# conceptofmind/vit-flax

Hardware: NVIDIA B200
Metric: images/sec ViT-B/16 224 bf16 fwd at 1/2/4/8 B200; % tensor-pipe peak (higher is better)
Workload: dtype bf16

## Files before the change

vit_flax_b200/csrc/attention_tc5.cu:

```cuda
#include <cstdlib>

#include "common.h"
#include "ptx.cuh"

namespace vb {

#ifdef VITB200_TRACE
__device__ long long g_trace[12][64];
#define TRACE(ev, i) do { if (blockIdx.x == 0 && (i) < 64) g_trace[ev][i] = clock64(); } while (0)
#else
#define TRACE(ev, i) do { } while (0)
#endif

namespace {

constexpr int DH = 64;
constexpr int QT = 128;
constexpr int NT = 512;
constexpr int Q_BYTES = QT * 128;
constexpr int O_BYTES = QT * 128;

constexpr int QS = 4;
constexpr int KS = 2;

// ... 26 lines not shown
        fma_f32x2(pack_f32x2(__uint_as_float(r[2 * j]), __uint_as_float(r[2 * j + 1])), sl2x2, mnegx2);
    float a0, a1;
    unpack_f32x2(a2, a0, a1);
    const float p0 = ex2_approx(a0), p1 = ex2_approx(a1);
    if (j & 1) lb = add_f32x2(lb, pack_f32x2(p0, p1));
    else la = add_f32x2(la, pack_f32x2(p0, p1));
    pp[j] = pack2<kDT>(p0, p1);
  }
}

template <int kDT, int KP>
__global__ void __launch_bounds__(NT, 1)
attention_tc5_kernel(const __grid_constant__ CUtensorMap tmQ,
                     const __grid_constant__ CUtensorMap tmKV,
                     const __grid_constant__ CUtensorMap tmO,
                     int T, int heads, int nqt, int items, int turns, float* __restrict__ lse_out) {
  using L = Smem<KP>;
  constexpr uint32_t SLOT_COLS = KP <= 128 ? 128 : 208;
  constexpr uint32_t O_COL = 2 * SLOT_COLS;
  static_assert(O_COL + DH <= 512, "TMEM budget");
  extern __shared__ uint8_t smem_raw[];
  const uint32_t base = (smem_u32(smem_raw) + 1023u) & ~1023u;
  uint8_t* gbase = smem_raw + (base - smem_u32(smem_raw));
  const uint32_t sQ = base + L::OFF_Q, sK = base + L::OFF_K, sV = base + L::OFF_V, sO = base + L::OFF_O;
  const uint32_t bars = base + L::OFF_BAR;
  auto q_full = [&](int s) { return bars + 8u * (0 + s); };
  auto q_empty = [&](int s) { return bars + 8u * (4 + s); };
  auto k_full = [&](int s) { return bars + 8u * (8 + s); };
  auto v_full = [&](int s) { return bars + 8u * (10 + s); };
  auto k_empty = [&](int s) { return bars + 8u * (12 + s); };
  auto v_empty = [&](int s) { return bars + 8u * (14 + s); };
// ... 14 lines not shown
  const int n = int(last - first);

  if (warp == 0 && lane == 0) {
    prefetch_tmap(&tmQ);
    prefetch_tmap(&tmKV);
    prefetch_tmap(&tmO);
  }
  if (warp == 1 && lane == 0) {
    for (int s = 0; s < QS; ++s) {
      mbar_init(q_full(s), 1);
      mbar_init(q_empty(s), 1);
    }
    for (int s = 0; s < 2; ++s) {
      mbar_init(k_full(s), 1);
      mbar_init(v_full(s), 1);
      mbar_init(k_empty(s), nqt);
      mbar_init(v_empty(s), nqt);
      mbar_init(s_ready(s), 1);
      for (int g = 0; g < 4; ++g) mbar_init(p_part(s, g), 4);
      mbar_init(o_ready(s), 1);
    }
    mbar_init(o_free, 4);
    for (int q = 0; q < 4; ++q) mbar_init(xu_done(q), 1);
    fence_barrier_init();
  }
  if (warp == 2) tmem_alloc<1>(tmem_slot, 512);
  tc_fence_before();
  __syncthreads();
  tc_fence_after();
  const uint32_t tmem_base = *tmem_slot_ptr;
  pdl_launch_dependents();
  pdl_wait();

  const int bh0 = int(first / nqt);
  if (warp == 0) {
    if (elect_one()) {
      for (int i = 0; i < n; ++i) {
        const int64_t item = first + i;
        const int bh = int(item / nqt), qt = int(item - int64_t(bh) * nqt);
        const int b = bh / heads, h = bh - b * heads;
        const int e = bh - bh0, es = e & 1;
        const uint32_t eph = (e >> 1) & 1;
        const bool first_of_bh = (i == 0) || (qt == 0);
        if (first_of_bh) {
          mbar_wait(k_empty(es), eph ^ 1u);
          mbar_arrive_expect_tx(k_full(es), L::KV_BYTES);
          tma_load_3d(sK + es * L::KV_BYTES, &tmKV, k_full(es), inner + h * DH, 0, b);
        }
        const int qs = i & (QS - 1);
        mbar_wait(q_empty(qs), ((i / QS) & 1) ^ 1u);
        TRACE(0, i);
        mbar_arrive_expect_tx(q_full(qs), Q_BYTES);
        tma_load_3d(sQ + qs * Q_BYTES, &tmQ, q_full(qs), h * DH, qt * QT, b);
        if (first_of_bh) {
          mbar_wait(v_empty(es), eph ^ 1u);
          TRACE(1, i);
          mbar_arrive_expect_tx(v_full(es), L::KV_BYTES);
          tma_load_3d(sV + es * L::KV_BYTES, &tmKV, v_full(es), 2 * inner + h * DH, 0, b);
        }
      }
    }
    __syncwarp();
  } else if (warp == 1 || warp == 3) {
    if (elect_one()) {
      constexpr int fmt = kDT == DT_F16 ? 0 : 1;
      constexpr uint32_t idesc_s = umma_idesc_16(QT, KP, fmt, 0);
      constexpr uint32_t idesc_o = umma_idesc_16(QT, DH, fmt, 1);
      constexpr int NPARTS = KP >= 128 ? KP / 64 : 1;
      const int s = warp == 1 ? 0 : 1;
      const uint32_t d_s = tmem_base + s * SLOT_COLS, d_o = tmem_base + O_COL;
      const int first_lo = int(first % nqt);
      auto meta = [&](int i, int& es, uint32_t& eph, int& missing) {
        const int t = first_lo + i;
        const int e = t / nqt;
        es = e & 1;
        eph = (e >> 1) & 1;
        missing = i == 0 ? first_lo : 0;
      };
      auto issue_s = [&](int i) {
        int es, missing; uint32_t eph;
        meta(i, es, eph, missing);
        const int qs = i & (QS - 1);
        mbar_wait(q_full(qs), (i / QS) & 1);
        mbar_wait(k_full(es), eph);
        TRACE(2, i);
        tc_fence_after();
        const uint32_t q0 = sQ + qs * Q_BYTES, k0 = sK + es * L::KV_BYTES;
#pragma unroll
        for (int k = 0; k < DH / 16; ++k)
          umma_bf16_ss<1>(d_s, umma_desc_k_sw128(q0 + k * 32), umma_desc_k_sw128(k0 + k * 32), idesc_s,
                          k != 0 ? 1u : 0u);
        umma_commit(q_empty(qs));
        umma_commit(k_empty(es));
        for (int j = 0; j < missing; ++j) mbar_arrive(k_empty(es));
        umma_commit(s_ready(s));
      };
      if (s < n) issue_s(s);
      for (int i = s; i < n; i += 2) {
        int es, missing; uint32_t eph;
        meta(i, es, eph, missing);
        const uint32_t ph = (i >> 1) & 1;
        const uint32_t v0 = sV + es * L::KV_BYTES;
#pragma unroll
        for (int g = 0; g < NPARTS; ++g) {
          mbar_wait(p_part(s, g), ph);
          if (g == 0) {
            mbar_wait(v_full(es), eph);
            mbar_wait(o_free, uint32_t(i & 1) ^ 1u);
            TRACE(3, i);
          }
          tc_fence_after();
          constexpr int KSTEPS = KP / 16;
          const int k_end = g == NPARTS - 1 ? KSTEPS : 4 * g + 4;
#pragma unroll
          for (int kk = 4 * g; kk < k_end; ++kk)
            umma_bf16_ts(d_o, d_s + kk * 8, umma_desc_mn_sw128(v0 + kk * 2048), idesc_o, kk != 0 ? 1u : 0u);
        }
        umma_commit(v_empty(es));
        for (int j = 0; j < missing; ++j) mbar_arrive(v_empty(es));
        umma_commit(o_ready(s));
        if (i + 2 < n) issue_s(i + 2);
      }
    }
    __syncwarp();
  } else if (warp >= 4 && warp < 12) {
    const int w = warp - 4;
    const int q = w & 3;
    const int grp = w >> 2;
    const int row = q * 32 + lane;
    const uint32_t t_slot = tmem_base + (uint32_t(q * 32) << 16) + uint32_t(grp * SLOT_COLS);
    const float sl2 = 0.125f * 1.4426950408889634f;
    constexpr int NFULL = KP / 32, TAIL = KP % 32;
    constexpr int KMIN = KP == 208 ? 128 : (KP == 128 ? 64 : 0);
    static_assert(TAIL == 0 || TAIL == 16, "key block = n*32 (+16)");
    constexpr int NPARTS = KP >= 128 ? KP / 64 : 1;
    static_assert(NPARTS <= 4 && 2 * NPARTS <= NFULL, "parts are pairs of 32-key chunks");

    for (int i = grp; i < n; i += 2) {
      const uint32_t ph = (i >> 1) & 1;
      const int64_t item = first + i;
      const int bh = int(item / nqt), qt = int(item - int64_t(bh) * nqt);
      const bool active = qt * QT + q * 32 < T;
      if (q == 0 && lane == 0) TRACE(4, i);
      mbar_wait(s_ready(grp), ph);
      if (q == 0 && lane == 0) TRACE(5, i);
      tc_fence_after();
      if (active) {
        uint32_t r[2][32];
        float mx = -INFINITY;
        tmem_ld_32x32b_x32p(t_slot, r[0]);
        tmem_ld_wait();
#pragma unroll
        for (int c = 0; c < NFULL; ++c) {
          if (c + 1 < NFULL) tmem_ld_32x32b_x32p(t_slot + (c + 1) * 32, r[(c + 1) & 1]);
          else if (TAIL) tmem_ld_32x32b_x16(t_slot + (c + 1) * 32, r[(c + 1) & 1]);
          uint32_t* rc = r[c & 1];
          if (c * 32 + 32 > KMIN && c * 32 + 32 > T) {
// ... 38 lines not shown
            if (lane == 0) mbar_arrive(p_part(grp, c / 2 - 1));
          }
          tmem_st_32x32b_x16(t_slot + c * 16, pp);
          if (c + 1 == turns) { __syncwarp(); if (lane == 0) mbar_arrive(xu_done(q)); }
        }
        if constexpr (TAIL != 0) {
          uint32_t pp[8];
          softmax_chunk<kDT, 16, true>(r[NFULL & 1], pp, NFULL * 32, T, sl2x2, mnegx2, la, lb);
          tmem_st_32x32b_x8(t_slot + NFULL * 16, pp);
        }
        if (turns > NFULL) { __syncwarp(); if (lane == 0) mbar_arrive(xu_done(q)); }
        if (q == 0 && lane == 0) TRACE(11, i);
        float l0, l1;
        unpack_f32x2(add_f32x2(la, lb), l0, l1);
        inv_sh[(i & 3) * 128 + row] = 1.0f / (l0 + l1);
        if (lse_out != nullptr && qt * QT + row < T) lse_out[int64_t(bh) * T + qt * QT + row] = __log2f(l0 + l1) - mneg;
        tmem_st_wait();
        tc_fence_before();
        __syncwarp();
        if (lane == 0) mbar_arrive(p_part(grp, NPARTS - 1));
      } else {
        if (turns) {
          mbar_wait(xu_done(q), uint32_t(i & 1) ^ 1u);
          if (lane == 0) mbar_arrive(xu_done(q));
        }
        tc_fence_before();
        __syncwarp();
        if (lane == 0) {
#pragma unroll
          for (int g = 0; g < NPARTS; ++g) mbar_arrive(p_part(grp, g));
        }
      }
      if (q == 0 && lane == 0) TRACE(7, i);
    }
  } else if (warp >= 12) {
    const int q = warp & 3;
    const int row = q * 32 + lane;
    const bool leader = (q == 0 && lane == 0);
    const uint32_t t_lane = tmem_base + (uint32_t(q * 32) << 16);
    for (int i = 0; i < n; ++i) {
      const int s = i & 1;
      const uint32_t ph = (i >> 1) & 1;
      const int64_t item = first + i;
      const int bh = int(item / nqt), qt = int(item - int64_t(bh) * nqt);
      const int b = bh / heads, h = bh - b * heads;
      const bool active = qt * QT + q * 32 < T;
      const uint32_t sOi = sO + uint32_t(i & 1) * O_BYTES;
      if (leader) TRACE(8, i);
      mbar_wait(o_ready(s), ph);
      tc_fence_after();
      uint32_t o[64];
      float inv = 0.f;
      if (active) {
        tmem_ld_32x32b_x32p(t_lane + O_COL, o);
        tmem_ld_32x32b_x32p(t_lane + O_COL + 32, o + 32);
        inv = inv_sh[(i & 3) * 128 + row];
        tmem_ld_wait();
      }
      tc_fence_before();
      __syncwarp();
      if (lane == 0) mbar_arrive(o_free);
      if (active) {
#pragma unroll
        for (int g = 0; g < 8; ++g) {
          st_shared_v4(sOi + uint32_t(row) * 128u + (uint32_t(g ^ (row & 7)) << 4),
                       pack2<kDT>(__uint_as_float(o[g * 8 + 0]) * inv, __uint_as_float(o[g * 8 + 1]) * inv),
                       pack2<kDT>(__uint_as_float(o[g * 8 + 2]) * inv, __uint_as_float(o[g * 8 + 3]) * inv),
                       pack2<kDT>(__uint_as_float(o[g * 8 + 4]) * inv, __uint_as_float(o[g * 8 + 5]) * inv),
                       pack2<kDT>(__uint_as_float(o[g * 8 + 6]) * inv, __uint_as_float(o[g * 8 + 7]) * inv));
        }
      }
      fence_proxy_async_smem();
      if (leader) tma_store_wait_read<0>();
      named_bar_sync(1, 128);
      if (leader) {
        tma_store_3d(&tmO, sOi, h * DH, qt * QT, b);
        tma_store_commit();
        TRACE(10, i);
      }
    }
    if (leader) tma_store_wait<0>();
  }

  tc_fence_before();
  __syncthreads();
  if (warp == 2) {
    tc_fence_after();
    tmem_dealloc<1>(tmem_base, 512);
  }
}

int attn_turns() {
  static int v = -1;
  if (v < 0) {
    const char* e = getenv("VITB200_ATTN_TURNS");
    v = (e && e[0] >= '0' && e[0] <= '9') ? e[0] - '0' : -1;
  }
  return v;
}

template <int kDT, int KP>
int launch_kp(cudaStream_t stream, const void* qkv, void* out, int batch, int T, int heads, float* lse, int q_tiles) {
  using L = Smem<KP>;
  static PerDevice<bool> configured_on;
  if (bool& configured = configured_on.here(); !configured) {
    VB_CUDA(cudaFuncSetAttribute(attention_tc5_kernel<kDT, KP>, cudaFuncAttributeMaxDynamicSharedMemorySize, L::TOTAL));
    configured = true;
  }
  const int inner = heads * DH;
  CUtensorMap tq, tkv, to;
  int rc;
  if ((rc = make_tmap_3d_16(&tq, qkv, batch, T, 3 * inner, 3 * inner, QT, kDT))) return rc;
  if ((rc = make_tmap_3d_16(&tkv, qkv, batch, T, 3 * inner, 3 * inner, KP, kDT))) return rc;
  if ((rc = make_tmap_3d_16(&to, out, batch, T, inner, inner, QT, kDT))) return rc;
  const int nqt = q_tiles > 0 && q_tiles < ceil_div(T, QT) ? q_tiles : ceil_div(T, QT);
  const int64_t items64 = int64_t(batch) * heads * nqt;
  if (items64 > 0x7fffffff) return fail(VITB200_ERR_INVALID, "attention: too many work items");
  const int items = int(items64);
  const int grid = items < sm_count() ? items : sm_count();
  VB_CUDA(launch_kernel(attention_tc5_kernel<kDT, KP>, dim3(grid), dim3(NT), L::TOTAL, stream, 1,
                        tq, tkv, to, T, heads, nqt, items, attn_turns(), lse));
  VB_LAUNCH_CHECK("attention_tc5_kernel");
  return 0;
}

template <int kDT>
int launch_dt(cudaStream_t stream, const void* qkv, void* out, int batch, int T, int heads, float* lse, int q_tiles) {
  if (T <= 64) return launch_kp<kDT, 64>(stream, qkv, out, batch, T, heads, lse, q_tiles);
  if (T <= 128) return launch_kp<kDT, 128>(stream, qkv, out, batch, T, heads, lse, q_tiles);
  return launch_kp<kDT, 208>(stream, qkv, out, batch, T, heads, lse, q_tiles);
}

}

#ifdef VITB200_TRACE
}
extern "C" int vitb200_debug_attention_trace(long long* host, int n) {
  return cudaMemcpyFromSymbol(host, vb::g_trace, sizeof(long long) * (n < 12 * 64 ? n : 12 * 64)) == cudaSuccess ? 0 : -2;
}
namespace vb {
#endif

bool attention_tc5_supports(int T) { return T >= 1 && T <= 208; }

int launch_attention_tc5(cudaStream_t stream, const void* qkv, void* out, int batch, int T, int heads,
// ... 10 lines not shown
```

vit_flax_b200/csrc/common.h:

```cpp
#pragma once
#include <cuda.h>
#include <cuda_runtime.h>
#include <cuda_bf16.h>
#include <stdint.h>
#include <string>

#include "../../include/vitb200.h"
#include "ptx.cuh"

namespace vb {

void set_error(const std::string& msg);
int fail(int code, const std::string& msg);
int cuda_fail(cudaError_t e, const char* what);
void count_launch(int n = 1);
const std::string& last_error_ref();
int64_t launch_count();

#define VB_CUDA(expr)                                              \
  do {                                                             \
    cudaError_t _e = (expr);                                       \
    if (_e != cudaSuccess) return ::vb::cuda_fail(_e, #expr);      \
  } while (0)

// ... 38 lines not shown
    ++na;
  }
  if (pdl_enabled()) {
    attr[na].id = cudaLaunchAttributeProgrammaticStreamSerialization;
    attr[na].val.programmaticStreamSerializationAllowed = 1;
    ++na;
  }
  cfg.attrs = attr;
  cfg.numAttrs = unsigned(na);
  return cudaLaunchKernelEx(&cfg, kernel, KArgs(args)...);
}

int make_tmap_2d(CUtensorMap* out, const void* base, int64_t rows, int64_t cols, int64_t ld,
                 int box_rows, int dt, int box_bytes = 128);
int make_tmap_3d_16(CUtensorMap* out, const void* base, int64_t batch, int64_t rows, int64_t cols,
                    int64_t ld, int box_rows, int dt);

int make_tmap_im2col_patches(CUtensorMap* out, const float* images, int64_t batch, int H, int W, int C, int ph, int pw,
                             int pixels);

constexpr int GEMM_BM = 128;
constexpr int GEMM_BN = 256;
constexpr int GEMM_BK = 64;

int launch_gemm_tc(cudaStream_t stream, const CUtensorMap& tmA, const CUtensorMap& tmB,
                   const CUtensorMap* tmC, const float* bias, void* C, int M, int N, int K,
                   int epilogue, const float* aux, int tokens_per_image, int dtype, int cta_group,
                   const Dropout& drop = Dropout(), int cls_off = 1, const float* cls = nullptr,
                   const LnFold& ln = LnFold(), const float* wscale = nullptr);
int launch_fold_layernorm(cudaStream_t stream, const float* W, const float* gamma, const float* beta, const float* bias,
                          void* Wt, float* c, float* d, int K, int N, int Kpad, int dtype, float* scratch);
// ... 92 lines not shown
```

vit_flax_b200/csrc/ptx.cuh:

```cuda
#pragma once
#include <cuda_runtime.h>
#include <cuda_bf16.h>
#include <cuda_fp16.h>
#include <stdint.h>
#include <stdio.h>

namespace vb {

__device__ __forceinline__ uint32_t smem_u32(const void* p) {
  return static_cast<uint32_t>(__cvta_generic_to_shared(p));
}
__device__ __forceinline__ uint32_t lane_id() { return threadIdx.x & 31u; }
__device__ __forceinline__ bool elect_one() {
  uint32_t pred;
  asm volatile("{\n\t.reg .pred p;\n\telect.sync _|p, 0xffffffff;\n\tselp.u32 %0, 1, 0, p;\n\t}" : "=r"(pred));
  return pred != 0;
}

__device__ __forceinline__ void pdl_wait() { asm volatile("griddepcontrol.wait;" ::: "memory"); }
__device__ __forceinline__ void pdl_launch_dependents() {
  asm volatile("griddepcontrol.launch_dependents;" ::: "memory");
}

__device__ __forceinline__ void mbar_init(uint32_t bar, uint32_t count) {
// ... 107 lines not shown
  asm volatile("cp.async.bulk.tensor.2d.global.shared::cta.bulk_group [%0, {%2, %3}], [%1];"
               ::"l"(reinterpret_cast<uint64_t>(tmap)), "r"(src), "r"(c0), "r"(c1) : "memory");
}
__device__ __forceinline__ void tma_reduce_add_2d(const void* tmap, uint32_t src, int32_t c0, int32_t c1) {
  asm volatile("cp.reduce.async.bulk.tensor.2d.global.shared::cta.add.tile.bulk_group [%0, {%2, %3}], [%1];"
               ::"l"(reinterpret_cast<uint64_t>(tmap)), "r"(src), "r"(c0), "r"(c1) : "memory");
}
__device__ __forceinline__ void tma_store_3d(const void* tmap, uint32_t src, int32_t c0, int32_t c1, int32_t c2) {
  asm volatile("cp.async.bulk.tensor.3d.global.shared::cta.bulk_group [%0, {%2, %3, %4}], [%1];"
               ::"l"(reinterpret_cast<uint64_t>(tmap)), "r"(src), "r"(c0), "r"(c1), "r"(c2) : "memory");
}
__device__ __forceinline__ void tma_load_3d(uint32_t dst, const void* tmap, uint32_t bar,
                                            int32_t c0, int32_t c1, int32_t c2) {
  asm volatile(
      "cp.async.bulk.tensor.3d.shared::cluster.global.mbarrier::complete_tx::bytes"
      " [%0], [%1, {%3, %4, %5}], [%2];"
      ::"r"(dst), "l"(reinterpret_cast<uint64_t>(tmap)), "r"(bar), "r"(c0), "r"(c1), "r"(c2)
      : "memory");
}
__device__ __forceinline__ void tma_load_im2col_5d(uint32_t dst, const void* tmap, uint32_t bar, int32_t c, int32_t w,
                                                   int32_t h, int32_t d, int32_t n, uint16_t w_off, uint16_t h_off,
                                                   uint16_t d_off) {
  asm volatile(
      "cp.async.bulk.tensor.5d.shared::cluster.global.im2col.mbarrier::complete_tx::bytes"
      " [%0], [%1, {%3, %4, %5, %6, %7}], [%2], {%8, %9, %10};"
      ::"r"(dst), "l"(reinterpret_cast<uint64_t>(tmap)), "r"(bar), "r"(c), "r"(w), "r"(h), "r"(d), "r"(n), "h"(w_off),
        "h"(h_off), "h"(d_off)
      : "memory");
}
__device__ __forceinline__ void tma_store_commit() { asm volatile("cp.async.bulk.commit_group;" ::: "memory"); }
// ... 164 lines not shown

__device__ __forceinline__ uint64_t umma_desc_k_sw128(uint32_t addr) {
  return static_cast<uint64_t>((addr & 0x3FFFFu) >> 4)
         | (1ull << 16)
         | (64ull << 32)
         | (1ull << 46)
         | (2ull << 61);
}
__device__ __forceinline__ uint64_t umma_desc_mn_sw128(uint32_t addr) {
  return static_cast<uint64_t>((addr & 0x3FFFFu) >> 4) | (1ull << 16) | (64ull << 32) |
         (1ull << 46) | (2ull << 61);
}
__device__ __forceinline__ uint64_t umma_desc_mn_sw128_wide(uint32_t addr, uint32_t lbo_bytes) {
  return static_cast<uint64_t>((addr & 0x3FFFFu) >> 4) | (static_cast<uint64_t>(lbo_bytes >> 4) << 16) |
         (64ull << 32) | (1ull << 46) | (2ull << 61);
}
constexpr uint32_t UMMA_DESC_HI_SW128 = 0x40004040u;
__device__ __forceinline__ uint32_t umma_desc_lo(uint32_t addr, uint32_t lbo_bytes = 16) {
  return ((addr & 0x3FFFFu) >> 4) | ((lbo_bytes >> 4) << 16);
}
__device__ __forceinline__ void umma_bf16_ss_lo(uint32_t d_tmem, uint32_t a_lo, uint32_t b_lo, uint32_t idesc, uint32_t accumulate) {
  asm volatile(
      "{\n\t.reg .pred p;\n\t.reg .b64 da, db;\n\t"
      "setp.ne.b32 p, %4, 0;\n\t"
      "mov.b64 da, {%1, %5};\n\t"
      "mov.b64 db, {%2, %5};\n\t"
      "tcgen05.mma.cta_group::1.kind::f16 [%0], da, db, %3, p;\n\t}"
      ::"r"(d_tmem), "r"(a_lo), "r"(b_lo), "r"(idesc), "r"(accumulate), "r"(UMMA_DESC_HI_SW128) : "memory");
}

// ... 131 lines not shown
```

vit_flax_b200/csrc/runtime.cu:

```cuda
#include <atomic>
#include <cstdlib>
#include <mutex>

#include "common.h"

namespace vb {

namespace {
thread_local std::string g_last_error;
std::atomic<int64_t> g_launches{0};

typedef CUresult (*EncodeTiledFn)(CUtensorMap*, CUtensorMapDataType, cuuint32_t, void*,
                                  const cuuint64_t*, const cuuint64_t*, const cuuint32_t*,
                                  const cuuint32_t*, CUtensorMapInterleave, CUtensorMapSwizzle,
                                  CUtensorMapL2promotion, CUtensorMapFloatOOBfill);
EncodeTiledFn g_encode = nullptr;
std::once_flag g_encode_once;
typedef CUresult (*EncodeIm2colFn)(CUtensorMap*, CUtensorMapDataType, cuuint32_t, void*, const cuuint64_t*,
                                   const cuuint64_t*, const int*, const int*, cuuint32_t, cuuint32_t, const cuuint32_t*,
                                   CUtensorMapInterleave, CUtensorMapSwizzle, CUtensorMapL2promotion, CUtensorMapFloatOOBfill);
EncodeIm2colFn g_encode_im2col = nullptr;
std::once_flag g_encode_im2col_once;
}

// ... 60 lines not shown
  if (box_rows < 1 || box_rows > 256) return fail(VITB200_ERR_INVALID, "TMA box rows out of range");
  if (box_bytes != 128 && box_bytes != 64) return fail(VITB200_ERR_INVALID, "TMA box width must be 64 or 128 bytes");
  cuuint64_t gdim[2] = {static_cast<cuuint64_t>(cols), static_cast<cuuint64_t>(rows)};
  cuuint64_t gstride[1] = {static_cast<cuuint64_t>(ld) * esz};
  cuuint32_t box[2] = {static_cast<cuuint32_t>(box_bytes / esz), static_cast<cuuint32_t>(box_rows)};
  cuuint32_t estr[2] = {1u, 1u};
  CUresult r = g_encode(out, tmap_type(dt), 2, const_cast<void*>(base), gdim, gstride, box, estr,
                        CU_TENSOR_MAP_INTERLEAVE_NONE, box_bytes == 64 ? CU_TENSOR_MAP_SWIZZLE_64B : CU_TENSOR_MAP_SWIZZLE_128B,
                        CU_TENSOR_MAP_L2_PROMOTION_L2_256B, CU_TENSOR_MAP_FLOAT_OOB_FILL_NONE);
  if (r != CUDA_SUCCESS)
    return fail(VITB200_ERR_CUDA, "cuTensorMapEncodeTiled failed with CUresult " + std::to_string(int(r)));
  return 0;
}

int make_tmap_3d_16(CUtensorMap* out, const void* base, int64_t batch, int64_t rows, int64_t cols,
                    int64_t ld, int box_rows, int dt) {
  if (!load_encoder()) return fail(VITB200_ERR_CUDA, "cuTensorMapEncodeTiled entry point unavailable");
  if ((reinterpret_cast<uintptr_t>(base) & 15) != 0 || (ld * 2) % 16 != 0)
    return fail(VITB200_ERR_INVALID, "TMA operand must be 16-byte aligned with a 16-byte row pitch");
  if (box_rows < 1 || box_rows > 256) return fail(VITB200_ERR_INVALID, "TMA box rows out of range");
  cuuint64_t gdim[3] = {static_cast<cuuint64_t>(cols), static_cast<cuuint64_t>(rows), static_cast<cuuint64_t>(batch)};
  cuuint64_t gstride[2] = {static_cast<cuuint64_t>(ld) * 2, static_cast<cuuint64_t>(ld) * 2 * static_cast<cuuint64_t>(rows)};
  cuuint32_t box[3] = {64u, static_cast<cuuint32_t>(box_rows), 1u};
  cuuint32_t estr[3] = {1u, 1u, 1u};
  CUresult r = g_encode(out, tmap_type(dt), 3, const_cast<void*>(base), gdim, gstride, box, estr,
                        CU_TENSOR_MAP_INTERLEAVE_NONE, CU_TENSOR_MAP_SWIZZLE_128B,
                        CU_TENSOR_MAP_L2_PROMOTION_L2_256B, CU_TENSOR_MAP_FLOAT_OOB_FILL_NONE);
  if (r != CUDA_SUCCESS)
    return fail(VITB200_ERR_CUDA, "cuTensorMapEncodeTiled(3d) failed with CUresult " + std::to_string(int(r)));
  return 0;
}

int make_tmap_im2col_patches(CUtensorMap* out, const float* images, int64_t batch, int H, int W, int C, int ph, int pw,
                             int pixels) {
  std::call_once(g_encode_im2col_once, [] {
    void* fn = nullptr;
    cudaDriverEntryPointQueryResult q;
    if (cudaGetDriverEntryPoint("cuTensorMapEncodeIm2col", &fn, cudaEnableDefault, &q) == cudaSuccess &&
        q == cudaDriverEntryPointSuccess)
      g_encode_im2col = reinterpret_cast<EncodeIm2colFn>(fn);
  });
// ... 22 lines not shown
```

Baseline: 28840.

## Add two-CTA cluster attention kernel splitting each head across a CTA pair

Adds an attention kernel for ViT's 197-token sequences in which a two-CTA cluster handles one (batch, head). It uses cta_group::2 UMMA with M=256: each CTA loads half of K and half of V's columns, and P is staged through shared memory for the PV product. The existing single-CTA kernel loses its multi-q-tile path and now does one q tile per head item; the pair kernel runs whenever q_tiles != 1. The aim is to avoid the duplicated K/V loads and the partial second q tile of the per-q-tile scheme and to use the larger 2-SM MMA shape. The cost is cross-CTA mbarrier synchronisation and new SW32/SW64 descriptor layouts, which bring correctness risk.

```diff
diff --git a/vit_flax_b200/csrc/attention_tc5.cu b/vit_flax_b200/csrc/attention_tc5.cu
--- a/vit_flax_b200/csrc/attention_tc5.cu
+++ b/vit_flax_b200/csrc/attention_tc5.cu
@@ -64,7 +64,7 @@
 attention_tc5_kernel(const __grid_constant__ CUtensorMap tmQ,
                      const __grid_constant__ CUtensorMap tmKV,
                      const __grid_constant__ CUtensorMap tmO,
-                     int T, int heads, int nqt, int items, int turns, float* __restrict__ lse_out) {
+                     int T, int heads, int items, int turns, float* __restrict__ lse_out) {
   using L = Smem<KP>;
   constexpr uint32_t SLOT_COLS = KP <= 128 ? 128 : 208;
   constexpr uint32_t O_COL = 2 * SLOT_COLS;
@@ -109,8 +109,8 @@
     for (int s = 0; s < 2; ++s) {
       mbar_init(k_full(s), 1);
       mbar_init(v_full(s), 1);
-      mbar_init(k_empty(s), nqt);
-      mbar_init(v_empty(s), nqt);
+      mbar_init(k_empty(s), 1);
+      mbar_init(v_empty(s), 1);
       mbar_init(s_ready(s), 1);
       for (int g = 0; g < 4; ++g) mbar_init(p_part(s, g), 4);
       mbar_init(o_ready(s), 1);
@@ -127,32 +127,24 @@
   pdl_launch_dependents();
   pdl_wait();
 
-  const int bh0 = int(first / nqt);
   if (warp == 0) {
     if (elect_one()) {
       for (int i = 0; i < n; ++i) {
-        const int64_t item = first + i;
-        const int bh = int(item / nqt), qt = int(item - int64_t(bh) * nqt);
-        const int b = bh / heads, h = bh - b * heads;
-        const int e = bh - bh0, es = e & 1;
-        const uint32_t eph = (e >> 1) & 1;
-        const bool first_of_bh = (i == 0) || (qt == 0);
-        if (first_of_bh) {
-          mbar_wait(k_empty(es), eph ^ 1u);
-          mbar_arrive_expect_tx(k_full(es), L::KV_BYTES);
-          tma_load_3d(sK + es * L::KV_BYTES, &tmKV, k_full(es), inner + h * DH, 0, b);
-        }
+        const int bh = int(first + i), b = bh / heads, h = bh - b * heads;
+        const int es = i & 1;
+        const uint32_t eph = (i >> 1) & 1;
+        mbar_wait(k_empty(es), eph ^ 1u);
+        mbar_arrive_expect_tx(k_full(es), L::KV_BYTES);
+        tma_load_3d(sK + es * L::KV_BYTES, &tmKV, k_full(es), inner + h * DH, 0, b);
         const int qs = i & (QS - 1);
         mbar_wait(q_empty(qs), ((i / QS) & 1) ^ 1u);
         TRACE(0, i);
         mbar_arrive_expect_tx(q_full(qs), Q_BYTES);
-        tma_load_3d(sQ + qs * Q_BYTES, &tmQ, q_full(qs), h * DH, qt * QT, b);
-        if (first_of_bh) {
-          mbar_wait(v_empty(es), eph ^ 1u);
-          TRACE(1, i);
-          mbar_arrive_expect_tx(v_full(es), L::KV_BYTES);
-          tma_load_3d(sV + es * L::KV_BYTES, &tmKV, v_full(es), 2 * inner + h * DH, 0, b);
-        }
+        tma_load_3d(sQ + qs * Q_BYTES, &tmQ, q_full(qs), h * DH, 0, b);
+        mbar_wait(v_empty(es), eph ^ 1u);
+        TRACE(1, i);
+        mbar_arrive_expect_tx(v_full(es), L::KV_BYTES);
+        tma_load_3d(sV + es * L::KV_BYTES, &tmKV, v_full(es), 2 * inner + h * DH, 0, b);
       }
     }
     __syncwarp();
@@ -164,43 +156,30 @@
       constexpr int NPARTS = KP >= 128 ? KP / 64 : 1;
       const int s = warp == 1 ? 0 : 1;
       const uint32_t d_s = tmem_base + s * SLOT_COLS, d_o = tmem_base + O_COL;
-      const int first_lo = int(first % nqt);
-      auto meta = [&](int i, int& es, uint32_t& eph, int& missing) {
-        const int t = first_lo + i;
-        const int e = t / nqt;
-        es = e & 1;
-        eph = (e >> 1) & 1;
-        missing = i == 0 ? first_lo : 0;
-      };
       auto issue_s = [&](int i) {
-        int es, missing; uint32_t eph;
-        meta(i, es, eph, missing);
         const int qs = i & (QS - 1);
         mbar_wait(q_full(qs), (i / QS) & 1);
-        mbar_wait(k_full(es), eph);
+        mbar_wait(k_full(s), (i >> 1) & 1);
         TRACE(2, i);
         tc_fence_after();
-        const uint32_t q0 = sQ + qs * Q_BYTES, k0 = sK + es * L::KV_BYTES;
+        const uint32_t q0 = sQ + qs * Q_BYTES, k0 = sK + s * L::KV_BYTES;
 #pragma unroll
         for (int k = 0; k < DH / 16; ++k)
           umma_bf16_ss<1>(d_s, umma_desc_k_sw128(q0 + k * 32), umma_desc_k_sw128(k0 + k * 32), idesc_s,
                           k != 0 ? 1u : 0u);
         umma_commit(q_empty(qs));
-        umma_commit(k_empty(es));
-        for (int j = 0; j < missing; ++j) mbar_arrive(k_empty(es));
+        umma_commit(k_empty(s));
         umma_commit(s_ready(s));
       };
       if (s < n) issue_s(s);
       for (int i = s; i < n; i += 2) {
-        int es, missing; uint32_t eph;
-        meta(i, es, eph, missing);
         const uint32_t ph = (i >> 1) & 1;
-        const uint32_t v0 = sV + es * L::KV_BYTES;
+        const uint32_t v0 = sV + s * L::KV_BYTES;
 #pragma unroll
         for (int g = 0; g < NPARTS; ++g) {
           mbar_wait(p_part(s, g), ph);
           if (g == 0) {
-            mbar_wait(v_full(es), eph);
+            mbar_wait(v_full(s), ph);
             mbar_wait(o_free, uint32_t(i & 1) ^ 1u);
             TRACE(3, i);
           }
@@ -211,8 +190,7 @@
           for (int kk = 4 * g; kk < k_end; ++kk)
             umma_bf16_ts(d_o, d_s + kk * 8, umma_desc_mn_sw128(v0 + kk * 2048), idesc_o, kk != 0 ? 1u : 0u);
         }
-        umma_commit(v_empty(es));
-        for (int j = 0; j < missing; ++j) mbar_arrive(v_empty(es));
+        umma_commit(v_empty(s));
         umma_commit(o_ready(s));
         if (i + 2 < n) issue_s(i + 2);
       }
@@ -233,9 +211,8 @@
 
     for (int i = grp; i < n; i += 2) {
       const uint32_t ph = (i >> 1) & 1;
-      const int64_t item = first + i;
-      const int bh = int(item / nqt), qt = int(item - int64_t(bh) * nqt);
-      const bool active = qt * QT + q * 32 < T;
+      const int bh = int(first + i);
+      const bool active = q * 32 < T;
       if (q == 0 && lane == 0) TRACE(4, i);
       mbar_wait(s_ready(grp), ph);
       if (q == 0 && lane == 0) TRACE(5, i);
@@ -304,7 +281,7 @@
         float l0, l1;
         unpack_f32x2(add_f32x2(la, lb), l0, l1);
         inv_sh[(i & 3) * 128 + row] = 1.0f / (l0 + l1);
-        if (lse_out != nullptr && qt * QT + row < T) lse_out[int64_t(bh) * T + qt * QT + row] = __log2f(l0 + l1) - mneg;
+        if (lse_out != nullptr && row < T) lse_out[int64_t(bh) * T + row] = __log2f(l0 + l1) - mneg;
         tmem_st_wait();
         tc_fence_before();
         __syncwarp();
@@ -331,10 +308,8 @@
     for (int i = 0; i < n; ++i) {
       const int s = i & 1;
       const uint32_t ph = (i >> 1) & 1;
-      const int64_t item = first + i;
-      const int bh = int(item / nqt), qt = int(item - int64_t(bh) * nqt);
-      const int b = bh / heads, h = bh - b * heads;
-      const bool active = qt * QT + q * 32 < T;
+      const int bh = int(first + i), b = bh / heads, h = bh - b * heads;
+      const bool active = q * 32 < T;
       const uint32_t sOi = sO + uint32_t(i & 1) * O_BYTES;
       if (leader) TRACE(8, i);
       mbar_wait(o_ready(s), ph);
@@ -364,7 +339,7 @@
       if (leader) tma_store_wait_read<0>();
       named_bar_sync(1, 128);
       if (leader) {
-        tma_store_3d(&tmO, sOi, h * DH, qt * QT, b);
+        tma_store_3d(&tmO, sOi, h * DH, 0, b);
         tma_store_commit();
         TRACE(10, i);
       }
@@ -380,6 +355,329 @@
   }
 }
 
+constexpr int PKP = 208;
+constexpr int PKH = PKP / 2;
+constexpr int PDV = DH / 2;
+struct PairSmem {
+  static constexpr int K_BYTES = PKH * 128;
+  static constexpr int V_BYTES = PKP * PDV * 2;
+  static constexpr int P_TAIL = 3 * QT * 128;
+  static constexpr int P_BYTES = P_TAIL + QT * 32;
+  static constexpr int OFF_Q = 0;
+  static constexpr int OFF_K = OFF_Q + 2 * Q_BYTES;
+  static constexpr int OFF_V = OFF_K + 2 * K_BYTES;
+  static constexpr int OFF_P = OFF_V + 2 * V_BYTES;
+  static constexpr int OFF_O = OFF_P + 2 * P_BYTES;
+  static constexpr int OFF_BAR = OFF_O + 2 * O_BYTES;
+  static constexpr int OFF_INV = OFF_BAR + 512;
+  static constexpr int TOTAL = OFF_INV + 4 * 128 * 4 + 1024 ;
+  static_assert(K_BYTES % 1024 == 0 && V_BYTES % 1024 == 0 && P_BYTES % 1024 == 0, "operand stages keep 1024-byte alignment");
+  static_assert(TOTAL <= 232448, "shared memory budget");
+};
+
+template <int kDT>
+__global__ void __launch_bounds__(NT, 1)
+attention_pair_kernel(const __grid_constant__ CUtensorMap tmQ,
+                      const __grid_constant__ CUtensorMap tmK,
+                      const __grid_constant__ CUtensorMap tmV,
+                      const __grid_constant__ CUtensorMap tmO,
+                      int T, int heads, int items, int turns, float* __restrict__ lse_out) {
+  using L = PairSmem;
+  constexpr int KP = PKP;
+  constexpr uint32_t SLOT_COLS = KP;
+  constexpr uint32_t O_COL = 2 * SLOT_COLS;
+  static_assert(O_COL + DH <= 512, "TMEM budget");
+  extern __shared__ uint8_t smem_raw[];
+  const uint32_t base = (smem_u32(smem_raw) + 1023u) & ~1023u;
+  uint8_t* gbase = smem_raw + (base - smem_u32(smem_raw));
+  const uint32_t sQ = base + L::OFF_Q, sK = base + L::OFF_K, sV = base + L::OFF_V, sP = base + L::OFF_P,
+                 sO = base + L::OFF_O;
+  const uint32_t bars = base + L::OFF_BAR;
+  auto q_full = [&](int s) { return bars + 8u * (0 + s); };
+  auto q_empty = [&](int s) { return bars + 8u * (2 + s); };
+  auto k_full = [&](int s) { return bars + 8u * (4 + s); };
+  auto k_empty = [&](int s) { return bars + 8u * (6 + s); };
+  auto v_full = [&](int s) { return bars + 8u * (8 + s); };
+  auto v_empty = [&](int s) { return bars + 8u * (10 + s); };
+  auto s_ready = [&](int s) { return bars + 8u * (12 + s); };
+  auto s_free = [&](int s) { return bars + 8u * (14 + s); };
+  auto o_ready = [&](int s) { return bars + 8u * (16 + s); };
+  const uint32_t o_free = bars + 8u * 18;
+  const uint32_t tmem_slot = bars + 8u * 24;
+  auto p_part = [&](int s, int g) { return bars + 8u * (32 + 4 * s + g); };
+  auto xu_done = [&](int q) { return bars + 8u * (40 + q); };
+  volatile uint32_t* tmem_slot_ptr = reinterpret_cast<volatile uint32_t*>(gbase + L::OFF_BAR + 8 * 24);
+  float* inv_sh = reinterpret_cast<float*>(gbase + L::OFF_INV);
+
+  const int warp = threadIdx.x >> 5, lane = threadIdx.x & 31;
+  const uint32_t rank = cluster_ctarank();
+  const int inner = heads * DH;
+  if (turns < 0) turns = KP / 32 - 1;
+  const int cluster = int(blockIdx.x >> 1), clusters = int(gridDim.x >> 1);
+  const int first = int(int64_t(cluster) * items / clusters);
+  const int n = int(int64_t(cluster + 1) * items / clusters) - first;
+  constexpr int NPARTS = KP / 64;
+
+  if (warp == 0 && lane == 0) {
+    prefetch_tmap(&tmQ);
+    prefetch_tmap(&tmK);
+    prefetch_tmap(&tmV);
+    prefetch_tmap(&tmO);
+  }
+  if (warp == 1 && lane == 0) {
+    for (int s = 0; s < 2; ++s) {
+      mbar_init(q_full(s), 1);
+      mbar_init(k_full(s), 1);
+      mbar_init(v_full(s), 1);
+      mbar_init(q_empty(s), 1);
+      mbar_init(k_empty(s), 1);
+      mbar_init(v_empty(s), 1);
+      mbar_init(s_ready(s), 1);
+      mbar_init(o_ready(s), 1);
+      mbar_init(s_free(s), 8);
+      for (int g = 0; g < NPARTS; ++g) mbar_init(p_part(s, g), 8);
+    }
+    mbar_init(o_free, 8);
+    for (int q = 0; q < 4; ++q) mbar_init(xu_done(q), 1);
+    fence_barrier_init();
+  }
+  if (warp == 2) tmem_alloc<2>(tmem_slot, 512);
+  tc_fence_before();
+  cluster_sync_all();
+  tc_fence_after();
+  const uint32_t tmem_base = *tmem_slot_ptr;
+  pdl_launch_dependents();
+  pdl_wait();
+
+  if (warp == 0) {
+    if (elect_one()) {
+      for (int i = 0; i < n; ++i) {
+        const int bh = first + i, b = bh / heads, h = bh - b * heads;
+        const int s = i & 1;
+        const uint32_t ph = (i >> 1) & 1;
+        mbar_wait(k_empty(s), ph ^ 1u);
+        if (rank == 0) mbar_arrive_expect_tx(k_full(s), 2 * L::K_BYTES);
+        tma_load_3d_cg2(sK + s * L::K_BYTES, &tmK, mapa_shared(k_full(s), 0), inner + h * DH, int(rank) * PKH, b);
+        mbar_wait(q_empty(s), ph ^ 1u);
+        if (rank == 0) mbar_arrive_expect_tx(q_full(s), 2 * Q_BYTES);
+        tma_load_3d_cg2(sQ + s * Q_BYTES, &tmQ, mapa_shared(q_full(s), 0), h * DH, int(rank) * QT, b);
+        mbar_wait(v_empty(s), ph ^ 1u);
+        if (rank == 0) mbar_arrive_expect_tx(v_full(s), 2 * L::V_BYTES);
+        tma_load_3d_cg2(sV + s * L::V_BYTES, &tmV, mapa_shared(v_full(s), 0), 2 * inner + h * DH + int(rank) * PDV, 0, b);
+      }
+    }
+    __syncwarp();
+  } else if (warp == 1 || warp == 3) {
+    if (rank == 0 && elect_one()) {
+      constexpr int fmt = kDT == DT_F16 ? 0 : 1;
+      constexpr uint32_t idesc_s = umma_idesc_16(2 * QT, KP, fmt, 0);
+      constexpr uint32_t idesc_o = umma_idesc_16(2 * QT, DH, fmt, 1);
+      constexpr uint16_t both = 0x3;
+      const int s = warp == 1 ? 0 : 1;
+      const uint32_t d_s = tmem_base + s * SLOT_COLS, d_o = tmem_base + O_COL;
+      const uint32_t p0 = sP + s * L::P_BYTES, v0 = sV + s * L::V_BYTES;
+      auto issue_s = [&](int i) {
+        const uint32_t ph = (i >> 1) & 1;
+        mbar_wait(q_full(s), ph);
+        mbar_wait(k_full(s), ph);
+        mbar_wait_cluster(s_free(s), ph ^ 1u);
+        tc_fence_after();
+        const uint32_t q0 = sQ + s * Q_BYTES, k0 = sK + s * L::K_BYTES;
+#pragma unroll
+        for (int k = 0; k < DH / 16; ++k)
+          umma_bf16_ss<2>(d_s, umma_desc_k_sw128(q0 + k * 32), umma_desc_k_sw128(k0 + k * 32), idesc_s, k != 0 ? 1u : 0u);
+        umma_commit_cg2_mc(q_empty(s), both);
+        umma_commit_cg2_mc(k_empty(s), both);
+        umma_commit_cg2_mc(s_ready(s), both);
+      };
+      if (s < n) issue_s(s);
+      for (int i = s; i < n; i += 2) {
+        const uint32_t ph = (i >> 1) & 1;
+#pragma unroll
+        for (int g = 0; g < NPARTS; ++g) {
+          if (g == NPARTS - 1 && i + 2 < n) issue_s(i + 2);
+          mbar_wait_cluster(p_part(s, g), ph);
+          if (g == 0) {
+            mbar_wait(v_full(s), ph);
+            mbar_wait_cluster(o_free, uint32_t(i & 1) ^ 1u);
+          }
+          tc_fence_after();
+          constexpr int KSTEPS = KP / 16;
+          const int k_end = g == NPARTS - 1 ? KSTEPS : 4 * g + 4;
+#pragma unroll
+          for (int kk = 4 * g; kk < k_end; ++kk) {
+            const uint64_t pdesc = kk < 12 ? umma_desc_k_sw128(p0 + (kk >> 2) * (QT * 128) + (kk & 3) * 32)
+                                           : umma_desc_k_sw32(p0 + L::P_TAIL);
+            umma_bf16_ss<2>(d_o, pdesc, umma_desc_mn_sw64(v0 + kk * 1024), idesc_o, kk != 0 ? 1u : 0u);
+          }
+        }
+        umma_commit_cg2_mc(v_empty(s), both);
+        umma_commit_cg2_mc(o_ready(s), both);
+      }
+    }
+    __syncwarp();
+  } else if (warp >= 4 && warp < 12) {
+    const int w = warp - 4;
+    const int q = w & 3;
+    const int grp = w >> 2;
+    const int row = q * 32 + lane;
+    const int qrow = int(rank) * QT + row;
+    const uint32_t t_slot = tmem_base + (uint32_t(q * 32) << 16) + uint32_t(grp * SLOT_COLS);
+    const uint32_t p_row = sP + grp * L::P_BYTES + uint32_t(row) * 128u;
+    const uint32_t p_tail = sP + grp * L::P_BYTES + L::P_TAIL + uint32_t(row) * 32u;
+    const uint32_t sw = uint32_t(row & 7), sw32 = uint32_t((row >> 2) & 1);
+    const bool active = int(rank) * QT + q * 32 < T;
+    const float sl2 = 0.125f * 1.4426950408889634f;
+    constexpr int NFULL = KP / 32, TAIL = KP % 32, KMIN = 128;
+    static_assert(TAIL == 16, "key block = 6 x 32 + 16");
+    auto publish = [&](uint32_t bar) {
+      fence_proxy_async_smem();
+      __syncwarp();
+      if (lane == 0) {
+        if (rank == 0) mbar_arrive(bar);
+        else mbar_arrive_remote(mapa_shared(bar, 0));
+      }
+    };
+    auto release_slot = [&]() {
+      tc_fence_before();
+      __syncwarp();
+      if (lane == 0) mbar_arrive_cluster(s_free(grp), 0);
+    };
+
+    for (int i = grp; i < n; i += 2) {
+      const uint32_t ph = (i >> 1) & 1;
+      const int bh = first + i;
+      mbar_wait(s_ready(grp), ph);
+      tc_fence_after();
+      if (active) {
+        uint32_t r[2][32];
+        float mx = -INFINITY;
+        tmem_ld_32x32b_x32p(t_slot, r[0]);
+        tmem_ld_wait();
+#pragma unroll
+        for (int c = 0; c < NFULL; ++c) {
+          if (c + 1 < NFULL) tmem_ld_32x32b_x32p(t_slot + (c + 1) * 32, r[(c + 1) & 1]);
+          else tmem_ld_32x32b_x16(t_slot + (c + 1) * 32, r[(c + 1) & 1]);
+          uint32_t* rc = r[c & 1];
+          if (c * 32 + 32 > KMIN && c * 32 + 32 > T) {
+#pragma unroll
+            for (int j = 0; j < 32; ++j)
+              if (c * 32 + j >= T) rc[j] = __float_as_uint(-INFINITY);
+          }
+#pragma unroll
+          for (int j = 0; j < 32; j += 2)
+            mx = fmaxf(mx, fmaxf(__uint_as_float(rc[j]), __uint_as_float(rc[j + 1])));
+          tmem_ld_wait();
+        }
+        {
+          uint32_t* rc = r[NFULL & 1];
+#pragma unroll
+          for (int j = 0; j < 16; ++j)
+            if (NFULL * 32 + j >= T) rc[j] = __float_as_uint(-INFINITY);
+#pragma unroll
+          for (int j = 0; j < 16; j += 2)
+            mx = fmaxf(mx, fmaxf(__uint_as_float(rc[j]), __uint_as_float(rc[j + 1])));
+        }
+        const float mneg = -mx * sl2;
+        const unsigned long long sl2x2 = pack_f32x2(sl2, sl2), mnegx2 = pack_f32x2(mneg, mneg);
+        unsigned long long la = pack_f32x2(0.f, 0.f), lb = la;
+        tmem_ld_32x32b_x32p(t_slot, r[0]);
+        tmem_ld_wait();
+        if (turns) mbar_wait(xu_done(q), uint32_t(i & 1) ^ 1u);
+        mbar_wait(o_ready(grp), ph ^ 1u);
+#pragma unroll
+        for (int c = 0; c < NFULL; ++c) {
+          if (c + 1 < NFULL) tmem_ld_32x32b_x32p(t_slot + (c + 1) * 32, r[(c + 1) & 1]);
+          else tmem_ld_32x32b_x16(t_slot + (c + 1) * 32, r[(c + 1) & 1]);
+          uint32_t pp[16];
+          if (c * 32 + 32 > KMIN && c * 32 + 32 > T) softmax_chunk<kDT, 32, true>(r[c & 1], pp, c * 32, T, sl2x2, mnegx2, la, lb);
+          else softmax_chunk<kDT, 32, false>(r[c & 1], pp, c * 32, T, sl2x2, mnegx2, la, lb);
+          tmem_ld_wait();
+          if (c == NFULL - 1) release_slot();
+          if (c >= 2 && (c & 1) == 0) publish(p_part(grp, c / 2 - 1));
+          const uint32_t blk = p_row + uint32_t(c >> 1) * (QT * 128);
+#pragma unroll
+          for (int t = 0; t < 4; ++t)
+            st_shared_v4(blk + (((uint32_t((c & 1) * 4 + t)) ^ sw) << 4), pp[4 * t], pp[4 * t + 1], pp[4 * t + 2], pp[4 * t + 3]);
+          if (c + 1 == turns) { __syncwarp(); if (lane == 0) mbar_arrive(xu_done(q)); }
+        }
+        {
+          uint32_t pp[8];
+          softmax_chunk<kDT, 16, true>(r[NFULL & 1], pp, NFULL * 32, T, sl2x2, mnegx2, la, lb);
+#pragma unroll
+          for (int t = 0; t < 2; ++t)
+            st_shared_v4(p_tail + ((uint32_t(t) ^ sw32) << 4), pp[4 * t], pp[4 * t + 1], pp[4 * t + 2], pp[4 * t + 3]);
+        }
+        if (turns > NFULL) { __syncwarp(); if (lane == 0) mbar_arrive(xu_done(q)); }
+        float l0, l1;
+        unpack_f32x2(add_f32x2(la, lb), l0, l1);
+        inv_sh[(i & 3) * 128 + row] = 1.0f / (l0 + l1);
+        if (lse_out != nullptr && qrow < T) lse_out[int64_t(bh) * T + qrow] = __log2f(l0 + l1) - mneg;
+        publish(p_part(grp, NPARTS - 1));
+      } else {
+        if (turns) {
+          mbar_wait(xu_done(q), uint32_t(i & 1) ^ 1u);
+          if (lane == 0) mbar_arrive(xu_done(q));
+        }
+        mbar_wait(o_ready(grp), ph ^ 1u);
+        release_slot();
+#pragma unroll
+        for (int g = 0; g < NPARTS; ++g) publish(p_part(grp, g));
+      }
+    }
+  } else if (warp >= 12) {
+    const int q = warp & 3;
+    const int row = q * 32 + lane;
+    const bool leader = (q == 0 && lane == 0);
+    const uint32_t t_lane = tmem_base + (uint32_t(q * 32) << 16);
+    const bool active = int(rank) * QT + q * 32 < T;
+    for (int i = 0; i < n; ++i) {
+      const int s = i & 1;
+      const uint32_t ph = (i >> 1) & 1;
+      const int bh = first + i, b = bh / heads, h = bh - b * heads;
+      const uint32_t sOi = sO + uint32_t(i & 1) * O_BYTES;
+      mbar_wait(o_ready(s), ph);
+      tc_fence_after();
+      uint32_t o[64];
+      float inv = 0.f;
+      if (active) {
+        tmem_ld_32x32b_x32p(t_lane + O_COL, o);
+        tmem_ld_32x32b_x32p(t_lane + O_COL + 32, o + 32);
+        inv = inv_sh[(i & 3) * 128 + row];
+        tmem_ld_wait();
+      }
+      tc_fence_before();
+      __syncwarp();
+      if (lane == 0) mbar_arrive_cluster(o_free, 0);
+      if (active) {
+#pragma unroll
+        for (int g = 0; g < 8; ++g) {
+          st_shared_v4(sOi + uint32_t(row) * 128u + (uint32_t(g ^ (row & 7)) << 4),
+                       pack2<kDT>(__uint_as_float(o[g * 8 + 0]) * inv, __uint_as_float(o[g * 8 + 1]) * inv),
+                       pack2<kDT>(__uint_as_float(o[g * 8 + 2]) * inv, __uint_as_float(o[g * 8 + 3]) * inv),
+                       pack2<kDT>(__uint_as_float(o[g * 8 + 4]) * inv, __uint_as_float(o[g * 8 + 5]) * inv),
+                       pack2<kDT>(__uint_as_float(o[g * 8 + 6]) * inv, __uint_as_float(o[g * 8 + 7]) * inv));
+        }
+      }
+      fence_proxy_async_smem();
+      if (leader) tma_store_wait_read<0>();
+      named_bar_sync(1, 128);
+      if (leader) {
+        tma_store_3d(&tmO, sOi, h * DH, int(rank) * QT, b);
+        tma_store_commit();
+      }
+    }
+    if (leader) tma_store_wait<0>();
+  }
+
+  tc_fence_before();
+  cluster_sync_all();
+  if (warp == 2) {
+    tc_fence_after();
+    tmem_dealloc<2>(tmem_base, 512);
+  }
+}
+
 int attn_turns() {
   static int v = -1;
   if (v < 0) {
@@ -390,7 +688,7 @@
 }
 
 template <int kDT, int KP>
-int launch_kp(cudaStream_t stream, const void* qkv, void* out, int batch, int T, int heads, float* lse, int q_tiles) {
+int launch_kp(cudaStream_t stream, const void* qkv, void* out, int batch, int T, int heads, float* lse) {
   using L = Smem<KP>;
   static PerDevice<bool> configured_on;
   if (bool& configured = configured_on.here(); !configured) {
@@ -403,22 +701,48 @@
   if ((rc = make_tmap_3d_16(&tq, qkv, batch, T, 3 * inner, 3 * inner, QT, kDT))) return rc;
   if ((rc = make_tmap_3d_16(&tkv, qkv, batch, T, 3 * inner, 3 * inner, KP, kDT))) return rc;
   if ((rc = make_tmap_3d_16(&to, out, batch, T, inner, inner, QT, kDT))) return rc;
-  const int nqt = q_tiles > 0 && q_tiles < ceil_div(T, QT) ? q_tiles : ceil_div(T, QT);
-  const int64_t items64 = int64_t(batch) * heads * nqt;
+  const int64_t items64 = int64_t(batch) * heads;
   if (items64 > 0x7fffffff) return fail(VITB200_ERR_INVALID, "attention: too many work items");
   const int items = int(items64);
   const int grid = items < sm_count() ? items : sm_count();
   VB_CUDA(launch_kernel(attention_tc5_kernel<kDT, KP>, dim3(grid), dim3(NT), L::TOTAL, stream, 1,
-                        tq, tkv, to, T, heads, nqt, items, attn_turns(), lse));
+                        tq, tkv, to, T, heads, items, attn_turns(), lse));
   VB_LAUNCH_CHECK("attention_tc5_kernel");
   return 0;
 }
 
 template <int kDT>
+int launch_pair(cudaStream_t stream, const void* qkv, void* out, int batch, int T, int heads, float* lse) {
+  using L = PairSmem;
+  static PerDevice<bool> configured_on;
+  if (bool& configured = configured_on.here(); !configured) {
+    VB_CUDA(cudaFuncSetAttribute(attention_pair_kernel<kDT>, cudaFuncAttributeMaxDynamicSharedMemorySize, L::TOTAL));
+    configured = true;
+  }
+  const int inner = heads * DH;
+  CUtensorMap tq, tk, tv, to;
+  int rc;
+  if ((rc = make_tmap_3d_16(&tq, qkv, batch, T, 3 * inner, 3 * inner, QT, kDT))) return rc;
+  if ((rc = make_tmap_3d_16(&tk, qkv, batch, T, 3 * inner, 3 * inner, PKH, kDT))) return rc;
+  if ((rc = make_tmap_3d_16(&tv, qkv, batch, T, 3 * inner, 3 * inner, PKP, kDT, 64))) return rc;
+  if ((rc = make_tmap_3d_16(&to, out, batch, T, inner, inner, QT, kDT))) return rc;
+  const int64_t items64 = int64_t(batch) * heads;
+  if (items64 > 0x7fffffff) return fail(VITB200_ERR_INVALID, "attention: too many work items");
+  const int items = int(items64);
+  const int pairs = sm_count() / 2;
+  const int clusters = items < pairs ? items : pairs;
+  VB_CUDA(launch_kernel(attention_pair_kernel<kDT>, dim3(2 * clusters), dim3(NT), L::TOTAL, stream, 2,
+                        tq, tk, tv, to, T, heads, items, attn_turns(), lse));
+  VB_LAUNCH_CHECK("attention_pair_kernel");
+  return 0;
+}
+
+template <int kDT>
 int launch_dt(cudaStream_t stream, const void* qkv, void* out, int batch, int T, int heads, float* lse, int q_tiles) {
-  if (T <= 64) return launch_kp<kDT, 64>(stream, qkv, out, batch, T, heads, lse, q_tiles);
-  if (T <= 128) return launch_kp<kDT, 128>(stream, qkv, out, batch, T, heads, lse, q_tiles);
-  return launch_kp<kDT, 208>(stream, qkv, out, batch, T, heads, lse, q_tiles);
+  if (T <= 64) return launch_kp<kDT, 64>(stream, qkv, out, batch, T, heads, lse);
+  if (T <= 128) return launch_kp<kDT, 128>(stream, qkv, out, batch, T, heads, lse);
+  if (q_tiles == 1) return launch_kp<kDT, 208>(stream, qkv, out, batch, T, heads, lse);
+  return launch_pair<kDT>(stream, qkv, out, batch, T, heads, lse);
 }
 
 }
diff --git a/vit_flax_b200/csrc/common.h b/vit_flax_b200/csrc/common.h
--- a/vit_flax_b200/csrc/common.h
+++ b/vit_flax_b200/csrc/common.h
@@ -76,7 +76,7 @@
 int make_tmap_2d(CUtensorMap* out, const void* base, int64_t rows, int64_t cols, int64_t ld,
                  int box_rows, int dt, int box_bytes = 128);
 int make_tmap_3d_16(CUtensorMap* out, const void* base, int64_t batch, int64_t rows, int64_t cols,
-                    int64_t ld, int box_rows, int dt);
+                    int64_t ld, int box_rows, int dt, int box_bytes = 128);
 
 int make_tmap_im2col_patches(CUtensorMap* out, const float* images, int64_t batch, int H, int W, int C, int ph, int pw,
                              int pixels);
diff --git a/vit_flax_b200/csrc/ptx.cuh b/vit_flax_b200/csrc/ptx.cuh
--- a/vit_flax_b200/csrc/ptx.cuh
+++ b/vit_flax_b200/csrc/ptx.cuh
@@ -145,6 +145,14 @@
                                             int32_t c0, int32_t c1, int32_t c2) {
   asm volatile(
       "cp.async.bulk.tensor.3d.shared::cluster.global.mbarrier::complete_tx::bytes"
+      " [%0], [%1, {%3, %4, %5}], [%2];"
+      ::"r"(dst), "l"(reinterpret_cast<uint64_t>(tmap)), "r"(bar), "r"(c0), "r"(c1), "r"(c2)
+      : "memory");
+}
+__device__ __forceinline__ void tma_load_3d_cg2(uint32_t dst, const void* tmap, uint32_t bar,
+                                                int32_t c0, int32_t c1, int32_t c2) {
+  asm volatile(
+      "cp.async.bulk.tensor.3d.cta_group::2.shared::cluster.global.mbarrier::complete_tx::bytes"
       " [%0], [%1, {%3, %4, %5}], [%2];"
       ::"r"(dst), "l"(reinterpret_cast<uint64_t>(tmap)), "r"(bar), "r"(c0), "r"(c1), "r"(c2)
       : "memory");
@@ -339,6 +347,12 @@
 __device__ __forceinline__ uint64_t umma_desc_mn_sw128_wide(uint32_t addr, uint32_t lbo_bytes) {
   return static_cast<uint64_t>((addr & 0x3FFFFu) >> 4) | (static_cast<uint64_t>(lbo_bytes >> 4) << 16) |
          (64ull << 32) | (1ull << 46) | (2ull << 61);
+}
+__device__ __forceinline__ uint64_t umma_desc_k_sw32(uint32_t addr) {
+  return static_cast<uint64_t>((addr & 0x3FFFFu) >> 4) | (1ull << 16) | (16ull << 32) | (1ull << 46) | (6ull << 61);
+}
+__device__ __forceinline__ uint64_t umma_desc_mn_sw64(uint32_t addr) {
+  return static_cast<uint64_t>((addr & 0x3FFFFu) >> 4) | (1ull << 16) | (32ull << 32) | (1ull << 46) | (4ull << 61);
 }
 constexpr uint32_t UMMA_DESC_HI_SW128 = 0x40004040u;
 __device__ __forceinline__ uint32_t umma_desc_lo(uint32_t addr, uint32_t lbo_bytes = 16) {
diff --git a/vit_flax_b200/csrc/runtime.cu b/vit_flax_b200/csrc/runtime.cu
--- a/vit_flax_b200/csrc/runtime.cu
+++ b/vit_flax_b200/csrc/runtime.cu
@@ -98,17 +98,18 @@
 }
 
 int make_tmap_3d_16(CUtensorMap* out, const void* base, int64_t batch, int64_t rows, int64_t cols,
-                    int64_t ld, int box_rows, int dt) {
+                    int64_t ld, int box_rows, int dt, int box_bytes) {
   if (!load_encoder()) return fail(VITB200_ERR_CUDA, "cuTensorMapEncodeTiled entry point unavailable");
   if ((reinterpret_cast<uintptr_t>(base) & 15) != 0 || (ld * 2) % 16 != 0)
     return fail(VITB200_ERR_INVALID, "TMA operand must be 16-byte aligned with a 16-byte row pitch");
   if (box_rows < 1 || box_rows > 256) return fail(VITB200_ERR_INVALID, "TMA box rows out of range");
+  if (box_bytes != 128 && box_bytes != 64) return fail(VITB200_ERR_INVALID, "TMA box width must be 64 or 128 bytes");
   cuuint64_t gdim[3] = {static_cast<cuuint64_t>(cols), static_cast<cuuint64_t>(rows), static_cast<cuuint64_t>(batch)};
   cuuint64_t gstride[2] = {static_cast<cuuint64_t>(ld) * 2, static_cast<cuuint64_t>(ld) * 2 * static_cast<cuuint64_t>(rows)};
-  cuuint32_t box[3] = {64u, static_cast<cuuint32_t>(box_rows), 1u};
+  cuuint32_t box[3] = {static_cast<cuuint32_t>(box_bytes / 2), static_cast<cuuint32_t>(box_rows), 1u};
   cuuint32_t estr[3] = {1u, 1u, 1u};
   CUresult r = g_encode(out, tmap_type(dt), 3, const_cast<void*>(base), gdim, gstride, box, estr,
-                        CU_TENSOR_MAP_INTERLEAVE_NONE, CU_TENSOR_MAP_SWIZZLE_128B,
+                        CU_TENSOR_MAP_INTERLEAVE_NONE, box_bytes == 64 ? CU_TENSOR_MAP_SWIZZLE_64B : CU_TENSOR_MAP_SWIZZLE_128B,
                         CU_TENSOR_MAP_L2_PROMOTION_L2_256B, CU_TENSOR_MAP_FLOAT_OOB_FILL_NONE);
   if (r != CUDA_SUCCESS)
     return fail(VITB200_ERR_CUDA, "cuTensorMapEncodeTiled(3d) failed with CUresult " + std::to_string(int(r)));
```

Measured after the change: 27540, median of 6. 4.5% lower.
